# tilmantroester/baryon_painter

Hardware: AMD Instinct MI355X
Metric: cvae_train_tiles_per_sec (higher is better)
Workload: dtype f32; 1 GPU; CVAE fiducial train step (fwd+bwd+Adam), batch 64/GPU of 512x512 tiles, fp32 (BASELINE.json configs[1]); tile=512, batch_per_gpu=64, global_batch=64, parallelism=dp1, batch_norm=single device, optimizer=FlatAdam(lr=1e-3) = torch.optim.Adam arithmetic, fused, schedule=weight gradients on a second HIP stream beside the rest of the backward pass

## Files before the change

baryon_painter_amd/_lib.py:

```python
import ctypes as C
import os

_HERE = os.path.dirname(os.path.abspath(__file__))
LIB_PATH = os.path.join(_HERE, "libbp_hip.so")

BP_OK = 0
BP_EINVAL, BP_EUNSUPPORTED, BP_ELAUNCH, BP_EWORKSPACE = -1, -2, -3, -4
IMPL_AUTO, IMPL_DIRECT, IMPL_MFMA, IMPL_BF16 = 0, 1, 2, 3
IMPL_SHARED = 0x100
IMPL_DEFER = 0x200
PACK_FWD, PACK_BWD = 0, 1
F32, BF16 = 0, 1
F64 = 2
RC_SHIFT_LOG, RC_LOG, RC_SHIFT_LOG_2P, RC_LOG_TANH, RC_X_1PX, RC_INV_X = range(6)


class View(C.Structure):
    _fields_ = [("ptr", C.c_void_p), ("n", C.c_int32), ("h", C.c_int32), ("w", C.c_int32),
                ("c", C.c_int32), ("cstride", C.c_int32), ("coff", C.c_int32), ("dtype", C.c_int32)]


class Pointwise(C.Structure):
    _fields_ = [("scale", C.c_void_p), ("shift", C.c_void_p), ("slope", C.c_void_p)]


class Conv(C.Structure):
    _fields_ = [("transposed", C.c_int32), ("cin", C.c_int32), ("cout", C.c_int32),
                ("k", C.c_int32), ("stride", C.c_int32), ("pad", C.c_int32), ("out_pad", C.c_int32)]


class BnTrain(C.Structure):
    _fields_ = [("count", C.c_double), ("gamma", C.c_void_p), ("beta", C.c_void_p), ("eps", C.c_float),
                ("momentum", C.c_float), ("running_mean", C.c_void_p), ("running_var", C.c_void_p),
                ("num_batches_tracked", C.c_void_p), ("scale", C.c_void_p), ("shift", C.c_void_p),
                ("save_mean", C.c_void_p), ("save_invstd", C.c_void_p)]


class BnBackwardFin(C.Structure):
    _fields_ = [("count", C.c_double), ("gamma", C.c_void_p), ("save_mean", C.c_void_p), ("save_invstd", C.c_void_p),
                ("param_grad_scale", C.c_float), ("dgamma", C.c_void_p), ("dbeta", C.c_void_p), ("coef_abc", C.c_void_p)]


class Latent(C.Structure):
    _fields_ = [("n", C.c_int32), ("L", C.c_int32), ("zc", C.c_int32), ("zh", C.c_int32),
                ("zw", C.c_int32), ("min_z_var", C.c_float)]


class Linear(C.Structure):
    _fields_ = [("in_features", C.c_int32), ("out_features", C.c_int32), ("in_c", C.c_int32), ("in_h", C.c_int32),
                ("in_w", C.c_int32), ("out_c", C.c_int32), ("out_h", C.c_int32), ("out_w", C.c_int32),
                ("has_bias", C.c_int32)]


class Loglik(C.Structure):
    _fields_ = [("n", C.c_int32), ("L", C.c_int32), ("c", C.c_int32), ("h", C.c_int32),
                ("w", C.c_int32), ("mu_softplus", C.c_int32), ("predict_var", C.c_int32),
                ("alpha_var", C.c_float), ("beta_kl", C.c_float), ("likelihood_scaling", C.c_float)]


_P = C.c_void_p
_VP = C.POINTER(View)
_PWP = C.POINTER(Pointwise)
_CP = C.POINTER(Conv)

SIGNATURES = {
    "bp_version": (C.c_int, []),
    "bp_set_option": (C.c_int, [C.c_char_p, C.c_int]),
    "bp_conv_ws_kind": (C.c_int, [_CP, C.c_int, _VP, _VP]),
    "bp_strerror": (C.c_char_p, [C.c_int]),
    "bp_conv_packed_floats": (C.c_int64, [_CP, C.c_int]),
    "bp_conv_kernel_id": (C.c_int, [_CP, C.c_int]),
    "bp_conv_pack": (C.c_int, [_CP, C.c_int, _P, _P, _P]),
    "bp_conv_pack_job_bytes": (C.c_int32, []),
    "bp_conv_pack_job": (C.c_int, [_CP, C.c_int, _P, _P, _P, C.POINTER(C.c_int64)]),
    "bp_conv_pack_jobs": (C.c_int, [_P, _P, C.c_int32, C.c_int64, _P]),
    "bp_conv_bf16_packed_elems": (C.c_int64, [_CP, C.c_int]),
    "bp_conv_bf16_pack": (C.c_int, [_CP, C.c_int, _P, _P, _P]),
    "bp_conv_bf16_supported": (C.c_int, [_CP, C.c_int, _VP, _VP]),
    "bp_conv_forward": (C.c_int, [_CP, _VP, _PWP, _P, _P, _P, _VP, C.c_int, _P]),
    "bp_conv_backward_data": (C.c_int, [_CP, _VP, _P, _P, _VP, C.c_int, _P]),
    "bp_conv_stats_workspace": (C.c_size_t, [_CP, C.c_int, _VP, _VP, C.c_int]),
    "bp_conv_forward_stats": (C.c_int, [_CP, _VP, _PWP, _P, _VP, _P, _P, C.c_size_t, C.c_int, _P]),
    "bp_conv_forward_bn": (C.c_int, [_CP, _VP, _PWP, _P, _VP, _P, C.POINTER(BnTrain), _P, C.c_size_t, C.c_int, _P]),
    "bp_conv_backward_data_stats": (C.c_int, [_CP, _VP, _P, _VP, _VP, _PWP, _P, _P, C.c_size_t, _P]),
    "bp_conv_backward_data_act_workspace": (C.c_size_t, [_CP, _VP, _VP]),
    "bp_conv_backward_data_act": (C.c_int, [_CP, _VP, _P, _VP, _VP, _PWP, _P, _P, C.c_size_t, _P]),
    "bp_conv_backward_weight_workspace": (C.c_size_t, [_CP, _VP, _VP]),
    "bp_conv_backward_weight": (C.c_int, [_CP, _VP, _PWP, _VP, _P, _P, _P, C.c_size_t, C.c_int, _P]),
    "bp_wgrad_defer_begin": (C.c_int, []),
    "bp_wgrad_defer_flush": (C.c_int, [C.c_int, _P]),
    "bp_peer_handle_bytes": (C.c_int, []),
    "bp_peer_max_doubles": (C.c_int, []),
    "bp_peer_create": (C.c_int, [C.c_int, C.c_int, C.POINTER(C.c_void_p), _P]),
    "bp_peer_open": (C.c_int, [_P, _P]),
    "bp_peer_all_reduce": (C.c_int, [_P, _P, C.c_int, C.c_int64, _P]),
    "bp_peer_status": (C.c_int64, [_P]),
    "bp_peer_bind": (C.c_int, [_P]),
    "bp_peer_slots": (C.c_int, []),
    "bp_peer_exchange_check": (C.c_int, [_P, _P, C.c_int, _P]),
    "bp_peer_destroy": (C.c_int, [_P]),
    "bp_channel_sums_workspace": (C.c_size_t, [_VP]),
    "bp_channel_sums": (C.c_int, [_VP, _P, _P, C.c_size_t, _P]),
    "bp_bn_finalize": (C.c_int, [_P, C.c_double, C.c_int32, _P, _P, C.c_float, C.c_float, _P, _P, _P,
                                 _P, _P, _P, _P, _P]),
    "bp_bn_eval_pointwise": (C.c_int, [C.c_int32, _P, _P, _P, _P, C.c_float, _P, _P, _P]),
    "bp_act_backward_workspace": (C.c_size_t, [_VP]),
    "bp_act_backward": (C.c_int, [_VP, _VP, _VP, _PWP, _VP, _VP, _P, _P, C.c_size_t, _P]),
    "bp_act_backward_bn": (C.c_int, [_VP, _VP, _VP, _PWP, _VP, _VP, _P, C.POINTER(BnBackwardFin), _P, C.c_size_t, _P]),
    "bp_bn_backward_finalize": (C.c_int, [_P, C.c_double, C.c_int32, _P, _P, _P, C.c_float, _P, _P, _P, _P]),
    "bp_bn_backward_apply": (C.c_int, [_VP, _VP, _P, _VP, _P]),
    "bp_act_bn_backward_apply": (C.c_int, [_VP, _VP, _VP, _PWP, _VP, _P, _VP, _P]),
    "bp_sums_to_float": (C.c_int, [_P, C.c_int32, _P, _P]),
    "bp_prelu_slope_grad": (C.c_int, [_P, C.c_int32, _P, _P]),
    "bp_residual_forward": (C.c_int, [_VP, _PWP, _VP, _PWP, C.c_float, _VP, _P]),
    "bp_nchw_to_view": (C.c_int, [_P, C.c_int32, _P, C.c_int32, _VP, _P]),
    "bp_view_to_nchw": (C.c_int, [_VP, _PWP, C.c_int32, _P, _P]),
    "bp_fill": (C.c_int, [_P, C.c_int64, C.c_float, _P]),
    "bp_repeat_samples": (C.c_int, [_VP, C.c_int32, _VP, _P]),
    "bp_repeat_samples_adjoint": (C.c_int, [_VP, C.c_int32, _VP, _P]),
    "bp_paint_load": (C.c_int, [_P, C.c_int32, _P, _P, C.c_int32, _VP, _P]),
    "bp_paint_load2": (C.c_int, [_P, C.c_int32, _P, _P, C.c_int32, _VP, _VP, _P]),
    "bp_paint_store": (C.c_int, [_VP, _PWP, C.c_int32, _P, _P, _P]),
    "bp_paint_load_mode": (C.c_int, [C.c_int32, _P, C.c_int32, _P, _P, C.c_int32, _VP, _P]),
    "bp_paint_load2_mode": (C.c_int, [C.c_int32, _P, C.c_int32, _P, _P, C.c_int32, _VP, _VP, _P]),
    "bp_paint_store_mode": (C.c_int, [C.c_int32, _VP, _PWP, C.c_int32, _P, _P, _P]),
    "bp_paint_load_cam": (C.c_int, [_P, C.c_int32, _P, _P, C.c_int32, _VP, _P]),
    "bp_paint_store_cam": (C.c_int, [_VP, _P, _P, _P]),
    "bp_split_scale_workspace": (C.c_size_t, [C.c_int32, C.c_int32, C.c_int32]),
    "bp_split_scale": (C.c_int, [_P, C.c_int32, C.c_int32, C.c_int32, C.c_int32, C.c_int32, _P, _P, _P, C.c_size_t,
                                 _VP, _P]),
    "bp_paint_load_scales2": (C.c_int, [_P, _P, _P, C.c_int32, C.c_int32, C.c_int32, _P, _P, _P, C.c_size_t, _VP, _VP,
                                        _P]),
    "bp_paint_store_scales": (C.c_int, [_VP, _PWP, C.c_int32, C.c_int32, _P, _P, _P]),
    "bp_paint_load_scales2_mode": (C.c_int, [C.c_int32, _P, _P, _P, C.c_int32, C.c_int32, C.c_int32, _P, _P, _P,
                                             C.c_size_t, _VP, _VP, _P]),
    "bp_paint_store_scales_mode": (C.c_int, [C.c_int32, _VP, _PWP, C.c_int32, C.c_int32, _P, _P, _P]),
    "bp_paint_store_fields": (C.c_int, [_P, C.c_int32, C.c_int32, C.c_int32, _VP, _PWP, C.c_int32, _P, _P, _P]),
    "bp_paint_store_moments": (C.c_int, [_P, C.c_int32, C.c_int32, C.c_int32, _VP, _PWP, C.c_int32, _P, C.c_int32, _P, _P,
                                         _P, _P]),
    "bp_philox_normal": (C.c_int, [C.c_uint64, _P, C.c_int32, C.c_int32, C.c_int32, _P, _P]),
    "bp_philox_normal_dev": (C.c_int, [_P, _P, C.c_int32, C.c_int32, C.c_int32, _P, _P]),
    "bp_likelihood_draw": (C.c_int, [_VP, C.c_int32, _VP, _P, _P, _P, _VP, _P]),
    "bp_plane_cut_workspace": (C.c_size_t, [C.c_int32, C.c_int32, C.c_int32]),
    "bp_plane_cut": (C.c_int, [_P, C.c_int32, C.c_int32, C.c_int32, _P, C.c_int32, C.c_int32, C.c_int32, _P,
                               C.c_size_t, _P, _P]),
    "bp_plane_blend": (C.c_int, [_P, C.c_int32, C.c_int32, _P, C.c_int32, C.c_int32, C.c_int32, C.c_int32, _P,
                                 C.c_int32, C.c_double, _P, _P, _P, C.c_int32, C.c_int32, _P]),
    "bp_plane_blend_fields": (C.c_int, [_P, C.c_int32, C.c_int32, C.c_int32, _P, C.c_int32, C.c_int32, C.c_int32,
                                        C.c_int32, _P, C.c_int32, C.c_double, _P, _P, _P, C.c_int32, C.c_int32, _P]),
    "bp_plane_finish": (C.c_int, [_P, _P, C.c_int64, _P, _P]),
    "bp_plane_project_order_workspace": (C.c_size_t, [C.c_int32, C.c_int32, C.c_int32]),
# ... 71 lines not shown
```

baryon_painter_amd/csrc/capi.hip:

```cpp
#include "common.hpp"
#include "kernels.hpp"
#include <cstring>

namespace {

bool conv_ok(const bp_conv* cv) {
  return cv && cv->cin > 0 && cv->cout > 0 && cv->k > 0 && cv->stride > 0 && cv->pad >= 0 && cv->out_pad >= 0 &&
         (cv->transposed == 0 || cv->transposed == 1) && (cv->transposed || cv->out_pad == 0) &&
         cv->out_pad < cv->stride + (cv->stride == 1);
}

bool shapes_ok(const bp_conv* cv, const bp_view* x, const bp_view* y, bool any = false) {
  if (any ? (!bp_view_ok_any(x) || !bp_view_ok_any(y)) : (!bp_view_ok(x) || !bp_view_ok(y))) return false;
  if (x->n != y->n || x->c != cv->cin || y->c != cv->cout) return false;
  return y->h == bp_conv_out_extent(cv, x->h) && y->w == bp_conv_out_extent(cv, x->w) && y->h > 0 && y->w > 0;
}

size_t align256(size_t v) { return (v + 255) & ~(size_t)255; }

}

struct WgradPrivateWs {
  explicit WgradPrivateWs(bool on) { bp_wgrad_private_ws(on); }
  ~WgradPrivateWs() { bp_wgrad_private_ws(false); }
};

extern "C" {

int bp_version(void) { return 100; }

int bp_set_option(const char* name, int value) {
  if (!name) return BP_EINVAL;
  if (!strcmp(name, "bf16_ws")) { bp_bf16_ws_set(value); return BP_OK; }
  if (!strcmp(name, "f32_ws")) { bp_f32_ws_set(value); return BP_OK; }
  if (!strcmp(name, "f32_wgrad_ws")) { bp_f32_wgrad_ws_set(value); return BP_OK; }
  if (!strcmp(name, "bf16_wgrad_ws")) { bp_bf16_wgrad_ws_set(value); return BP_OK; }
  return BP_EUNSUPPORTED;
}

const char* bp_strerror(int code) {
  switch (code) {
    case BP_OK: return "ok";
    case BP_EINVAL: return "invalid argument (null pointer or inconsistent shapes)";
    case BP_EUNSUPPORTED: return "shape not supported by the gfx950 kernels";
    case BP_ELAUNCH: return "kernel launch failed";
    case BP_EWORKSPACE: return "workspace missing or too small";
  }
  return "unknown error";
}

int64_t bp_conv_packed_floats(const bp_conv* cv, int dir) {
  if (!conv_ok(cv) || (dir != BP_PACK_FWD && dir != BP_PACK_BWD)) return -1;
  const ConvGeom g = dir == BP_PACK_FWD ? bp_geom_forward(cv) : bp_geom_backward_data(cv);
  return bp_igemm_packed_floats(g);
}

int bp_conv_kernel_id(const bp_conv* cv, int dir) {
  if (!conv_ok(cv) || (dir != BP_PACK_FWD && dir != BP_PACK_BWD)) return -1;
  return bp_igemm_kernel_id(dir == BP_PACK_FWD ? bp_geom_forward(cv) : bp_geom_backward_data(cv));
}

int bp_conv_pack(const bp_conv* cv, int dir, const float* w_torch, float* packed, void* stream) {
  if (!conv_ok(cv) || !w_torch || !packed || (dir != BP_PACK_FWD && dir != BP_PACK_BWD)) return BP_EINVAL;
  const ConvGeom g = dir == BP_PACK_FWD ? bp_geom_forward(cv) : bp_geom_backward_data(cv);
  return bp_igemm_pack(g, bp_wmap(cv, dir), w_torch, packed, bp_stream(stream));
}

int32_t bp_conv_pack_job_bytes(void) { return (int32_t)bp_igemm_pack_job_bytes(); }

int bp_conv_pack_job(const bp_conv* cv, int dir, const float* w_torch, float* packed, void* job, int64_t* nblocks) {
  if (!conv_ok(cv) || !w_torch || !packed || !job || !nblocks || (dir != BP_PACK_FWD && dir != BP_PACK_BWD))
    return BP_EINVAL;
  const ConvGeom g = dir == BP_PACK_FWD ? bp_geom_forward(cv) : bp_geom_backward_data(cv);
  return bp_igemm_pack_job(g, bp_wmap(cv, dir), w_torch, packed, job, nblocks);
}

int bp_conv_pack_jobs(const void* jobs_dev, const int64_t* first_block_dev, int32_t njobs, int64_t total_blocks,
                      void* stream) {
  if (!jobs_dev || !first_block_dev || njobs < 0 || total_blocks < 0) return BP_EINVAL;
  return bp_igemm_pack_jobs(jobs_dev, first_block_dev, njobs, total_blocks, bp_stream(stream));
}

int64_t bp_conv_bf16_packed_elems(const bp_conv* cv, int dir) {
  if (!conv_ok(cv) || (dir != BP_PACK_FWD && dir != BP_PACK_BWD)) return -1;
  return bp_bf16_packed_elems(dir == BP_PACK_FWD ? bp_geom_forward(cv) : bp_geom_backward_data(cv));
}

int bp_conv_bf16_pack(const bp_conv* cv, int dir, const float* w_torch, void* packed, void* stream) {
  if (!conv_ok(cv) || !w_torch || !packed || (dir != BP_PACK_FWD && dir != BP_PACK_BWD)) return BP_EINVAL;
  const ConvGeom g = dir == BP_PACK_FWD ? bp_geom_forward(cv) : bp_geom_backward_data(cv);
  return bp_bf16_pack(g, bp_wmap(cv, dir), w_torch, packed, bp_stream(stream));
}

int bp_conv_ws_kind(const bp_conv* cv, int dir, const bp_view* in, const bp_view* out) {
  if (!conv_ok(cv) || (dir != BP_PACK_FWD && dir != BP_PACK_BWD) || !bp_view_ok_any(in) || !bp_view_ok_any(out)) return 0;
  const ConvGeom g = dir == BP_PACK_FWD ? bp_geom_forward(cv) : bp_geom_backward_data(cv);
  if (in->dtype == BP_F32 && out->dtype == BP_F32) return bp_f32_ws_ok(g, in, out, nullptr, 0) ? 3 : 0;
  return bp_bf16_ws_ok(g, in, out, nullptr, 0) ? bp_bf16_ws_kind(g) : 0;
}

int bp_conv_bf16_supported(const bp_conv* cv, int dir, const bp_view* in, const bp_view* out) {
  if (!conv_ok(cv) || (dir != BP_PACK_FWD && dir != BP_PACK_BWD)) return 0;
  if ((in && !bp_view_ok_any(in)) || (out && !bp_view_ok_any(out))) return 0;
  return bp_bf16_igemm_ok(dir == BP_PACK_FWD ? bp_geom_forward(cv) : bp_geom_backward_data(cv), in, out) ? 1 : 0;
}

int bp_conv_forward(const bp_conv* cv, const bp_view* x, const bp_pointwise* x_pw, const float* packed_fwd,
                    const float* w_torch, const float* bias, const bp_view* y, int impl, void* stream) {
  if (!conv_ok(cv) || !shapes_ok(cv, x, y, impl == BP_IMPL_BF16)) return BP_EINVAL;
  const ConvGeom g = bp_geom_forward(cv);
  if (impl == BP_IMPL_BF16) {
    if (!packed_fwd) return BP_EINVAL;
    return bp_bf16_igemm_run(g, x, bp_pw(x_pw), packed_fwd, bias, y, bp_stream(stream));
  }
  if (impl == BP_IMPL_AUTO && packed_fwd) {
    const int rc = bp_igemm_run(g, x, bp_pw(x_pw), packed_fwd, bias, y, bp_stream(stream));
    if (rc != BP_EUNSUPPORTED || !w_torch) return rc;
    impl = BP_IMPL_DIRECT;
  }
  if (impl == BP_IMPL_AUTO) impl = BP_IMPL_DIRECT;
  if (impl == BP_IMPL_MFMA) {
    if (!packed_fwd) return BP_EINVAL;
    return bp_igemm_run(g, x, bp_pw(x_pw), packed_fwd, bias, y, bp_stream(stream));
  }
  if (!w_torch) return BP_EINVAL;
  return bp_direct_gather(g, bp_wmap(cv, BP_PACK_FWD), x, bp_pw(x_pw), w_torch, bias, y, bp_stream(stream));
}

size_t bp_conv_stats_workspace(const bp_conv* cv, int dir, const bp_view* x, const bp_view* y, int impl) {
  if (!conv_ok(cv) || !shapes_ok(cv, x, y, impl == BP_IMPL_BF16) || (dir != BP_PACK_FWD && dir != BP_PACK_BWD)) return 0;
  if (impl == BP_IMPL_BF16)
    return dir == BP_PACK_FWD ? bp_bf16_stats_workspace(bp_geom_forward(cv), x, y, 1)
                              : bp_bf16_stats_workspace(bp_geom_backward_data(cv), y, x, 2);
  return dir == BP_PACK_FWD ? bp_igemm_stats_workspace(bp_geom_forward(cv), x, y, 1)
                            : bp_igemm_stats_workspace(bp_geom_backward_data(cv), y, x, 2);
}

int bp_conv_forward_stats(const bp_conv* cv, const bp_view* x, const bp_pointwise* x_pw, const float* packed_fwd,
                          const bp_view* y, double* sums, void* workspace, size_t workspace_bytes, int impl,
                          void* stream) {
  if (!conv_ok(cv) || !shapes_ok(cv, x, y, impl == BP_IMPL_BF16) || !packed_fwd || !sums) return BP_EINVAL;
  const IgemmStatsReq sr{1, nullptr, PW{nullptr, nullptr, nullptr}, sums, workspace, workspace_bytes};
  if (impl == BP_IMPL_BF16)
    return bp_bf16_igemm_run(bp_geom_forward(cv), x, bp_pw(x_pw), packed_fwd, nullptr, y, bp_stream(stream), &sr);
  return bp_igemm_run(bp_geom_forward(cv), x, bp_pw(x_pw), packed_fwd, nullptr, y, bp_stream(stream), &sr);
}

int bp_conv_forward_bn(const bp_conv* cv, const bp_view* x, const bp_pointwise* x_pw, const float* packed_fwd,
                       const bp_view* y, double* sums, const bp_bn_train* bn, void* workspace, size_t workspace_bytes,
                       int impl, void* stream) {
  if (!conv_ok(cv) || !shapes_ok(cv, x, y, impl == BP_IMPL_BF16) || !packed_fwd || !sums || !bn || bn->count <= 0 ||
      !bn->scale || !bn->shift)
    return BP_EINVAL;
  const BnFin fin{bn->count, bn->gamma, bn->beta, bn->eps, bn->momentum, bn->running_mean, bn->running_var,
                  bn->num_batches_tracked, bn->scale, bn->shift, bn->save_mean, bn->save_invstd};
  const IgemmStatsReq sr{1, nullptr, PW{nullptr, nullptr, nullptr}, sums, workspace, workspace_bytes, &fin};
  if (impl == BP_IMPL_BF16)
    return bp_bf16_igemm_run(bp_geom_forward(cv), x, bp_pw(x_pw), packed_fwd, nullptr, y, bp_stream(stream), &sr);
  return bp_igemm_run(bp_geom_forward(cv), x, bp_pw(x_pw), packed_fwd, nullptr, y, bp_stream(stream), &sr);
}

int bp_conv_backward_data_stats(const bp_conv* cv, const bp_view* dy, const float* packed_bwd, const bp_view* dx,
                                const bp_view* x_raw, const bp_pointwise* x_pw, double* sums, void* workspace,
                                size_t workspace_bytes, void* stream) {
  const bool b16 = (dy && dy->dtype == BP_BF16) || (dx && dx->dtype == BP_BF16);
  if (!conv_ok(cv) || !shapes_ok(cv, dx, dy, b16) || !packed_bwd || !sums || !bp_view_ok_any(x_raw)) return BP_EINVAL;
  if (x_raw->n != dx->n || x_raw->h != dx->h || x_raw->w != dx->w || x_raw->c != dx->c) return BP_EINVAL;
  const IgemmStatsReq sr{2, x_raw, bp_pw(x_pw), sums, workspace, workspace_bytes};
  if (b16)
    return bp_bf16_igemm_run(bp_geom_backward_data(cv), dy, PW{nullptr, nullptr, nullptr}, packed_bwd, nullptr, dx,
                             bp_stream(stream), &sr);
  if (!bp_view_ok(x_raw)) return BP_EINVAL;
  return bp_igemm_run(bp_geom_backward_data(cv), dy, PW{nullptr, nullptr, nullptr}, packed_bwd, nullptr, dx,
                      bp_stream(stream), &sr);
}

size_t bp_conv_backward_data_act_workspace(const bp_conv* cv, const bp_view* dy, const bp_view* g) {
  const bool b16 = g && g->dtype == BP_BF16;
  if (!conv_ok(cv) || !shapes_ok(cv, g, dy, b16)) return 0;
  if (b16) return bp_bf16_stats_workspace(bp_geom_backward_data(cv), dy, g, 3);
  return bp_igemm_stats_workspace(bp_geom_backward_data(cv), dy, g, 3);
// ... 101 lines not shown
```

baryon_painter_amd/csrc/conv_flat.hip:

```cpp
#include "common.hpp"
#include "kernels.hpp"
#include <cstdlib>

namespace {

typedef float v4f __attribute__((ext_vector_type(4)));

constexpr int K = 7, CG = 8, CO = 16;
constexpr int NQ = CG / 4;
constexpr int NG = K * NQ;
constexpr int TH = 8, TW = 64;
constexpr int IH = TH + K - 1, IWP = TW + K - 1;
constexpr int PLANE = IH * IWP * 4;
constexpr int NU = IH * IWP * NQ;
constexpr int SL = (NU + 255) / 256;

struct FlatArgs {
  const float* in; int h, w, in_cs, in_co;
  float* out; int out_cs, out_co;
  const float* bias;
  const float* wp;
  PW pw;
  int n, tiles_x, tiles_y, i0, in_vec;
  const float* raw; int raw_cs, raw_co;
  PW spw;
  double* stat;
};

template <bool OUT_VEC, bool STATS2, bool RAW_VEC = true>
__global__ __launch_bounds__(256, 2) void flat_k7_kernel(FlatArgs a) {
  __shared__ __attribute__((aligned(16))) float tile[NQ * PLANE];
  __shared__ double lsum[STATS2 ? 8 * 256 : 1];
  __shared__ double red[STATS2 ? 4 : 1][2][CO];
  const int tid = threadIdx.x, lane = tid & 63;
  const int wave = __builtin_amdgcn_readfirstlane(tid >> 6);
  const int lm = lane & 15, kq = lane >> 4;

  float wreg[K][NG];
#pragma unroll
  for (int u = 0; u < K; ++u)
#pragma unroll
    for (int g = 0; g < NG; ++g) wreg[u][g] = a.wp[((u * NG + g) * 4 + kq) * CO + lm];
  v4f b4 = {0.f, 0.f, 0.f, 0.f};
  if (a.bias) b4 = v4f{a.bias[4 * kq], a.bias[4 * kq + 1], a.bias[4 * kq + 2], a.bias[4 * kq + 3]};

  if constexpr (STATS2) {
#pragma unroll
    for (int q = 0; q < 8; ++q) lsum[q * 256 + tid] = 0.0;
  }
  float ssc[STATS2 ? 4 : 1], ssf[STATS2 ? 4 : 1], ssl[STATS2 ? 4 : 1];
  if constexpr (STATS2) {
#pragma unroll
    for (int q = 0; q < 4; ++q) {
      const bool on = a.spw.scale != nullptr;
      ssc[q] = on ? a.spw.scale[4 * kq + q] : 1.f;
      ssf[q] = on ? a.spw.shift[4 * kq + q] : 0.f;
      ssl[q] = on ? a.spw.slope[4 * kq + q] : 1.f;
    }
  }
  const int q4 = tid % NQ;
  const PW4 p4 = pw4_load(a.pw, q4 * 4, CG);
  const int per_img = a.tiles_x * a.tiles_y;
  const int ntiles = per_img * a.n;
  float4 stage[SL];
  unsigned inside = 0;
  auto fetch = [&](int t) {
    const int n = t / per_img, r = t % per_img;
    const int y0 = (r / a.tiles_x) * TH + a.i0, x0 = (r % a.tiles_x) * TW + a.i0;
    const float* in_n = a.in + (int64_t)n * a.h * a.w * a.in_cs + a.in_co + q4 * 4;
    unsigned in = 0;
#pragma unroll
    for (int i = 0; i < SL; ++i) {
      const int e = tid + i * 256;
      const int pix = e / NQ, col = pix % IWP, row = pix / IWP;
      const int iy = y0 + row, ix = x0 + col;
      if (e < NU && iy >= 0 && iy < a.h && ix >= 0 && ix < a.w) in |= 1u << i;
      const int cy = min(max(iy, 0), a.h - 1), cx = min(max(ix, 0), a.w - 1);
      const float* p = in_n + ((int64_t)cy * a.w + cx) * a.in_cs;
      stage[i] = a.in_vec ? *reinterpret_cast<const float4*>(p) : make_float4(p[0], p[1], p[2], p[3]);
    }
    inside = in;
  };
  auto commit = [&]() {
#pragma unroll
    for (int i = 0; i < SL; ++i) {
// ... 1000 lines not shown
    auto frags = [&](int buf, int g) {
#pragma unroll
      for (int ii = 0; ii < 8; ++ii) {
        const int i = g * 8 + ii, j2 = i % 2, txp = (i / 2) % 8, ty = i / 16;
        const int off = j2 * HPLANE + ((ty * 2 + (txp & 1)) * HHALF + (txp >> 1)) * 4;
        f0[buf][ii] = base[off];
        f1[buf][ii] = base[off + 2 * HHALF * 4];
      }
    };
    frags(0, 0);
#pragma unroll
    for (int g = 0; g < HNW / 8; ++g) {
      if (g + 1 < HNW / 8) frags((g + 1) & 1, g + 1);
      if (g == 8) load_pw();
      __builtin_amdgcn_sched_barrier(0);
#pragma unroll
      for (int i = 0; i < 8; ++i) {
        acc0 = __builtin_amdgcn_mfma_f32_16x16x4f32(wreg[g * 8 + i], f0[g & 1][i], acc0, 0, 0, 0);
        acc1 = __builtin_amdgcn_mfma_f32_16x16x4f32(wreg[g * 8 + i], f1[g & 1][i], acc1, 0, 0, 0);
      }
      if (g < HSL) fetch_unit(g);
      if (g >= 9) finish_unit(g - 9);
      if (g < HSL || g >= 9) {
#pragma unroll
        for (int m = 0; m < 16; ++m) {
          __builtin_amdgcn_sched_group_barrier(0x008, 1, 0);
          __builtin_amdgcn_sched_group_barrier(0x002, 3, 0);
        }
      }
      __builtin_amdgcn_sched_barrier(0);
    }
    float4* xw = reinterpret_cast<float4*>(xch) + ((cur * 4 + rg) * 2) * 64 + lane;
    if (kh == 1) {
      xw[0] = make_float4(acc0[0], acc0[1], acc0[2], acc0[3]);
      xw[64] = make_float4(acc1[0], acc1[1], acc1[2], acc1[3]);
    }
    if (tn < ntiles) commit(tile + (cur ^ 1) * HTILE);
    __syncthreads();
    if (kh == 0) {
      const float4 u0 = xw[0], u1 = xw[64];
      acc0[0] += u0.x; acc0[1] += u0.y; acc0[2] += u0.z; acc0[3] += u0.w;
      acc1[0] += u1.x; acc1[1] += u1.y; acc1[2] += u1.z; acc1[3] += u1.w;
      const int c0 = 4 * (kq & 1);
      if (a.bias) {
#pragma unroll
        for (int q = 0; q < 4; ++q) { const float b = a.bias[c0 + q]; acc0[q] += b; acc1[q] += b; }
      }
      const int ox = ox0 + 2 * lm + (kq >> 1);
      float* out_n = a.out + (int64_t)n * a.h * a.w * a.out_cs + a.out_co + c0;
      if (ox < a.w) {
        if (oy0 < a.h)
          *reinterpret_cast<float4*>(out_n + ((int64_t)oy0 * a.w + ox) * a.out_cs) = make_float4(acc0[0], acc0[1], acc0[2], acc0[3]);
        if (oy0 + 1 < a.h)
          *reinterpret_cast<float4*>(out_n + ((int64_t)(oy0 + 1) * a.w + ox) * a.out_cs) = make_float4(acc1[0], acc1[1], acc1[2], acc1[3]);
      }
    }
    cur ^= 1;
  }
}

struct FlatHPackArgs { const float* w; float* dst; int64_t sa, sb; int flip; };
__global__ void flat_h7_pack_kernel(FlatHPackArgs a) {
  const int i = blockIdx.x * blockDim.x + threadIdx.x;
  if (i >= HKS * 64) return;
  const int m = i % 16, kq = (i / 16) % 4, k = i / 64;
  const int kh = k / HNW, ii = k % HNW;
  const int j = 2 * kh + ii % 2, txp = (ii / 2) % 8, ty = ii / 16;
  const int d = m / 8, co = m % 8, tx = txp - d, c = 4 * j + kq;
  float v = 0.f;
  if (tx >= 0 && tx < HK) {
    const int ky = a.flip ? HK - 1 - ty : ty, kx = a.flip ? HK - 1 - tx : tx;
    v = a.w[c * a.sa + co * a.sb + ky * HK + kx];
  }
  a.dst[i] = v;
}

}

static bool bp_flat_h7_ok(const ConvGeom& g) {
  static const bool off = getenv("BP_NOFLAT") != nullptr || getenv("BP_NOFLATH") != nullptr;
  return !off && g.k == HK && g.stride == 1 && g.pad == HPAD && g.cin_g == HCG && g.cout_g == HCO && g.nphase == 1;
}

static int64_t bp_flat_h7_packed_floats(const ConvGeom&) { return (int64_t)HKS * 64; }

static int bp_flat_h7_pack(const ConvGeom& g, const WeightMap& wm, const float* w_torch, float* packed, hipStream_t st) {
  FlatHPackArgs a{w_torch, packed, wm.sa, wm.sb, g.gather_transposed};
  hipLaunchKernelGGL(flat_h7_pack_kernel, dim3((HKS * 64 + 255) / 256), dim3(256), 0, st, a);
  BP_CHECK_LAUNCH();
  return BP_OK;
}

static int bp_flat_h7_run(const ConvGeom&, const bp_view* in, const PW& pw, const float* packed, const float* bias,
                          const bp_view* out, hipStream_t st, const IgemmStatsReq* sr) {
  if (sr || !bp_view_vec4(out)) return BP_EUNSUPPORTED;
  FlatHArgs a{};
  a.bias = bias;
  a.in = in->ptr; a.h = in->h; a.w = in->w; a.in_cs = in->cstride; a.in_co = in->coff;
  a.out = out->ptr; a.out_cs = out->cstride; a.out_co = out->coff;
  a.wp = packed; a.pw = pw; a.n = in->n; a.in_vec = bp_view_vec4(in) ? 1 : 0;
  a.tiles_x = bp_ceil_div(out->w, HTW); a.tiles_y = bp_ceil_div(out->h, HTH);
  const int64_t ntiles = (int64_t)a.tiles_x * a.tiles_y * a.n;
  if (ntiles > 0x7fffffff) return BP_EUNSUPPORTED;
  hipLaunchKernelGGL(flat_h7_kernel, dim3(flat_g4_grid((int)ntiles)), dim3(GNT), 0, st, a);
  BP_CHECK_LAUNCH();
  return BP_OK;
}

const ConvFamily& bp_family_flat() {
  static const ConvFamily f = {
      "flat", bp_flat_ok, bp_family_id<710000>, bp_flat_packed_floats, bp_flat_pack,
      [](const ConvGeom&, const bp_view*, const bp_view* out, int mode) { return bp_flat_stats_workspace(out, mode); },
      bp_flat_run, false};
  return f;
}
const ConvFamily& bp_family_flat_t4() {
  static const ConvFamily f = {  "flat_t4", bp_flat_t4_ok, bp_family_id<720000>, bp_flat_t4_packed_floats, bp_flat_t4_pack,
                                  bp_family_stats_mode1<bp_flat_t4_stats_workspace>, bp_flat_t4_run, false};
  return f;
}
const ConvFamily& bp_family_flat_g4() {
  static const ConvFamily f = {  "flat_g4", bp_flat_g4_ok, bp_family_id<730000>, bp_flat_g4_packed_floats, bp_flat_g4_pack,
                                  bp_family_stats_mode1<bp_flat_g4_stats_workspace>, bp_flat_g4_run, false};
  return f;
}
const ConvFamily& bp_family_flat_t64() {
  static const ConvFamily f = {  "flat_t64", bp_flat_t64_ok, bp_family_id<740000>, bp_flat_t64_packed_floats,
                                   bp_flat_t64_pack, bp_family_stats_mode1<bp_flat_t64_stats_workspace>, bp_flat_t64_run, false};
  return f;
}
const ConvFamily& bp_family_flat_h7() {
  static const ConvFamily f = {
      "flat_h7", bp_flat_h7_ok, bp_family_id<750000>, bp_flat_h7_packed_floats, bp_flat_h7_pack,
      [](const ConvGeom&, const bp_view*, const bp_view*, int) { return (size_t)0; }, bp_flat_h7_run, false};
  return f;
}
```

baryon_painter_amd/csrc/kernels.hpp:

```cpp
#pragma once
#include "common.hpp"

struct ConvFamily {
  const char* name;
  bool (*ok)(const ConvGeom& g);
  int (*kernel_id)(const ConvGeom& g);
  int64_t (*packed_floats)(const ConvGeom& g);
  int (*pack)(const ConvGeom& g, const WeightMap& wm, const float* w_torch, float* packed, hipStream_t st);
  size_t (*stats_workspace)(const ConvGeom& g, const bp_view* in, const bp_view* out, int mode);
  int (*run)(const ConvGeom& g, const bp_view* in, const PW& pw, const float* packed, const float* bias,
             const bp_view* out, hipStream_t st, const IgemmStatsReq* sr);
  bool batched_pack;
};
template <int ID>
int bp_family_id(const ConvGeom&) { return ID; }
template <size_t (*WS)(const bp_view* out)>
size_t bp_family_stats_mode1(const ConvGeom&, const bp_view*, const bp_view* out, int mode) { return mode == 1 ? WS(out) : 0; }

const ConvFamily& bp_family_enc();
const ConvFamily& bp_family_stem();
const ConvFamily& bp_family_flat();
const ConvFamily& bp_family_flat_t64();
const ConvFamily& bp_family_flat_t4();
const ConvFamily& bp_family_flat_g4();
const ConvFamily& bp_family_flat_h7();
const ConvFamily& bp_family_small();
const ConvFamily& bp_family_tiled();

int64_t bp_igemm_packed_floats(const ConvGeom& g);
int bp_igemm_kernel_id(const ConvGeom& g);
int bp_igemm_pack(const ConvGeom& g, const WeightMap& wm, const float* w_torch, float* packed, hipStream_t st);
int bp_igemm_pack_job(const ConvGeom& g, const WeightMap& wm, const float* w_torch, float* packed, void* job,
                      int64_t* nblocks);
int bp_igemm_run(const ConvGeom& g, const bp_view* in, const PW& pw, const float* packed, const float* bias,
                 const bp_view* out, hipStream_t st, const IgemmStatsReq* stats = nullptr);
size_t bp_igemm_stats_workspace(const ConvGeom& g, const bp_view* in, const bp_view* out, int mode);

size_t bp_igemm_pack_job_bytes();
int bp_igemm_tiled_pack_job(const ConvGeom& g, const WeightMap& wm, const float* w_torch, float* packed, void* job,
                            int64_t* nblocks);
int bp_igemm_pack_jobs(const void* jobs_dev, const int64_t* first_block_dev, int njobs, int64_t total_blocks,
                       hipStream_t st);
size_t bp_stats_rows_bytes(int64_t rows, int C);
int bp_stats_rows_finish(double* ws, int64_t rows, int C, const IgemmStatsReq* sr, hipStream_t st);
int bp_stats_row_stride(int n);
size_t bp_stats_rows_bytes_n(int64_t rows, int n);
int bp_stats_rows_finish_n(double* ws, int64_t rows, int n, const IgemmStatsReq* sr, hipStream_t st);

void bp_f32_ws_set(int v);
bool bp_f32_ws_ok(const ConvGeom& g, const bp_view* in, const bp_view* out, const float* bias, int stats_mode);
size_t bp_f32_ws_stats_workspace(const ConvGeom& g, const bp_view* out);
int bp_f32_ws_run(const ConvGeom& g, const bp_view* in, const PW& pw, const float* packed_tiled, const bp_view* out,
                  hipStream_t st, const IgemmStatsReq* sr);

int bp_direct_gather(const ConvGeom& g, const WeightMap& wm, const bp_view* in, const PW& pw, const float* w_torch,
                     const float* bias, const bp_view* out, hipStream_t st);
int bp_direct_wgrad(const bp_conv* cv, const bp_view* X, const PW& pwx, const bp_view* Y, const PW& pwy, float* dst,
                    hipStream_t st);

size_t bp_wgrad_mfma_workspace(const bp_conv* cv, const bp_view* X, const bp_view* Y);
int bp_wgrad_mfma(const bp_conv* cv, const bp_view* X, const PW& pwx, const bp_view* Y, const PW& pwy, float* dst,
                  void* workspace, size_t workspace_bytes, hipStream_t st, bool shared);
size_t bp_wgrad_bf16_workspace(const bp_conv* cv, const bp_view* X, const bp_view* Y);
int bp_wgrad_bf16_run(const bp_conv* cv, const bp_view* X, const PW& pwx, const bp_view* Y, const PW& pwy, float* dst,
                      void* workspace, size_t workspace_bytes, hipStream_t st);
void bp_wgrad_private_ws(bool on);
int bp_wgrad_defer_begin_impl();
int bp_wgrad_defer_flush_impl(hipStream_t st, int end);

using WgradPartialFn = int(const bp_conv* cv, const bp_view* X, const PW& pwx, const bp_view* Y, const PW& pwy, float* ws,
                           size_t ws_bytes, size_t* need, int* nsplit, int* cxp, int* cyp, hipStream_t st, bool dry);
WgradPartialFn bp_wgrad_ws_f32, bp_wgrad_enc, bp_wgrad_thin, bp_wgrad_small, bp_wgrad_tiles, bp_wgrad_bf16, bp_wgrad_ws_bf16;
void bp_f32_wgrad_ws_set(int v);
void bp_bf16_wgrad_ws_set(int v);
void bp_wgrad_tiles_target(int target);

bool bp_stem_wgrad_ok(const bp_conv* cv, const bp_view* X, const bp_view* Y, const PW& pwy, const float* dbias);
size_t bp_stem_wgrad_workspace(const bp_view* X);
int bp_stem_wgrad(const bp_view* X, const PW& pwx, const bp_view* Y, float* dst, void* workspace, size_t workspace_bytes,
                  hipStream_t st);
bool bp_wgrad_flat_ok(const bp_conv* cv, const bp_view* X, const bp_view* Y, const PW& pwy);
size_t bp_wgrad_flat_workspace(const bp_view* X);
int bp_wgrad_flat(const bp_view* X, const PW& pwx, const bp_view* Y, float* dst, void* workspace, size_t workspace_bytes,
                  hipStream_t st, bool shared);
bool bp_wgrad_flat_s2_ok(const bp_conv* cv, const bp_view* X, const bp_view* Y, const PW& pwx, const PW& pwy);
size_t bp_wgrad_flat_s2_workspace(const bp_view* Y);
int bp_wgrad_flat_s2(const bp_view* X, const PW& pwx, const bp_view* Y, const PW& pwy, float* dst, void* workspace,
                     size_t workspace_bytes, hipStream_t st, bool shared);

bool bp_bf16_igemm_ok(const ConvGeom& g, const bp_view* in, const bp_view* out);
int64_t bp_bf16_packed_elems(const ConvGeom& g);
int bp_bf16_pack(const ConvGeom& g, const WeightMap& wm, const float* w_torch, void* packed, hipStream_t st);
int bp_bf16_igemm_run(const ConvGeom& g, const bp_view* in, const PW& pw, const void* packed, const float* bias,
                      const bp_view* out, hipStream_t st, const IgemmStatsReq* stats = nullptr);
size_t bp_bf16_stats_workspace(const ConvGeom& g, const bp_view* in, const bp_view* out, int mode);

int64_t bp_bf16_flat_packed_elems(const ConvGeom& g);
int bp_bf16_flat_pack(const ConvGeom& g, const WeightMap& wm, const float* w_torch, uint16_t* dst, hipStream_t st);
bool bp_bf16_flat_ok(const ConvGeom& g, const bp_view* in, const bp_view* out, const float* bias, int stats);
size_t bp_bf16_flat_stats_workspace(const ConvGeom& g, const bp_view* in, const bp_view* out, int mode);
int bp_bf16_flat_run(const ConvGeom& g, const bp_view* in, const PW& pw, const uint16_t* packed_flat, const bp_view* out,
                     hipStream_t st, const IgemmStatsReq* sr);

void bp_bf16_ws_set(int v);
int bp_bf16_ws_kind(const ConvGeom& g);
int64_t bp_bf16_ws_packed_elems(const ConvGeom& g);
int bp_bf16_ws_pack(const ConvGeom& g, const WeightMap& wm, const float* w_torch, uint16_t* dst, hipStream_t st);
bool bp_bf16_ws_ok(const ConvGeom& g, const bp_view* in, const bp_view* out, const float* bias, int mode);
// ... 27 lines not shown
```

include/bp_hip.h:

```cpp
#ifndef BP_HIP_H
#define BP_HIP_H

#include <stddef.h>
#include <stdint.h>

#ifdef __cplusplus
extern "C" {
#endif

#define BP_OK 0
#define BP_EINVAL (-1)
#define BP_EUNSUPPORTED (-2)
#define BP_ELAUNCH (-3)
#define BP_EWORKSPACE (-4)

enum { BP_F32 = 0, BP_BF16 = 1 };

typedef struct bp_view {
  float* ptr;
  int32_t n, h, w;
  int32_t c;
  int32_t cstride;
  int32_t coff;
  int32_t dtype;
} bp_view;

typedef struct bp_pointwise {
  const float* scale;
  const float* shift;
  const float* slope;
} bp_pointwise;

typedef struct bp_conv {
  int32_t transposed;
  int32_t cin, cout;
  int32_t k, stride, pad, out_pad;
} bp_conv;

enum { BP_IMPL_AUTO = 0, BP_IMPL_DIRECT = 1, BP_IMPL_MFMA = 2, BP_IMPL_BF16 = 3 };
enum { BP_IMPL_SHARED = 0x100 };
enum { BP_IMPL_DEFER = 0x200 };
enum { BP_PACK_FWD = 0, BP_PACK_BWD = 1 };

int bp_version(void);
int bp_set_option(const char* name, int value);
const char* bp_strerror(int code);


int64_t bp_conv_packed_floats(const bp_conv* cv, int dir);

int bp_conv_kernel_id(const bp_conv* cv, int dir);

int bp_conv_pack(const bp_conv* cv, int dir, const float* w_torch, float* packed, void* stream);

int32_t bp_conv_pack_job_bytes(void);
int bp_conv_pack_job(const bp_conv* cv, int dir, const float* w_torch, float* packed, void* job,
                     int64_t* nblocks);
int bp_conv_pack_jobs(const void* jobs_dev, const int64_t* first_block_dev, int32_t njobs,
                      int64_t total_blocks, void* stream);

int64_t bp_conv_bf16_packed_elems(const bp_conv* cv, int dir);
int bp_conv_ws_kind(const bp_conv* cv, int dir, const bp_view* in, const bp_view* out);
int bp_conv_bf16_pack(const bp_conv* cv, int dir, const float* w_torch, void* packed, void* stream);
int bp_conv_bf16_supported(const bp_conv* cv, int dir, const bp_view* in, const bp_view* out);

int bp_conv_forward(const bp_conv* cv, const bp_view* x, const bp_pointwise* x_pw,
                    const float* packed_fwd, const float* w_torch, const float* bias,
                    const bp_view* y, int impl, void* stream);

int bp_conv_backward_data(const bp_conv* cv, const bp_view* dy, const float* packed_bwd,
                          const float* w_torch, const bp_view* dx, int impl, void* stream);

size_t bp_conv_stats_workspace(const bp_conv* cv, int dir, const bp_view* x, const bp_view* y, int impl);
int bp_conv_forward_stats(const bp_conv* cv, const bp_view* x, const bp_pointwise* x_pw, const float* packed_fwd,
                          const bp_view* y, double* sums, void* workspace, size_t workspace_bytes, int impl,
                          void* stream);
int bp_conv_backward_data_stats(const bp_conv* cv, const bp_view* dy, const float* packed_bwd, const bp_view* dx,
                                const bp_view* x_raw, const bp_pointwise* x_pw, double* sums, void* workspace,
                                size_t workspace_bytes, void* stream);

size_t bp_conv_backward_data_act_workspace(const bp_conv* cv, const bp_view* dy, const bp_view* g);
int bp_conv_backward_data_act(const bp_conv* cv, const bp_view* dy, const float* packed_bwd, const bp_view* g,
                              const bp_view* x_raw, const bp_pointwise* x_pw, double* sums, void* workspace,
                              size_t workspace_bytes, void* stream);

typedef struct bp_bn_train {
  double count;
  const float* gamma; const float* beta;
  float eps, momentum;
  float* running_mean; float* running_var; int64_t* num_batches_tracked;
  float* scale; float* shift;
  double* save_mean; double* save_invstd;
} bp_bn_train;
int bp_conv_forward_bn(const bp_conv* cv, const bp_view* x, const bp_pointwise* x_pw, const float* packed_fwd,
                       const bp_view* y, double* sums, const bp_bn_train* bn, void* workspace, size_t workspace_bytes,
                       int impl, void* stream);

size_t bp_conv_backward_weight_workspace(const bp_conv* cv, const bp_view* x, const bp_view* dy);
int bp_conv_backward_weight(const bp_conv* cv, const bp_view* x, const bp_pointwise* x_pw,
                            const bp_view* dy, float* dw_torch, float* dbias, void* workspace,
                            size_t workspace_bytes, int impl, void* stream);

int bp_wgrad_defer_begin(void);
int bp_wgrad_defer_flush(int end, void* stream);


size_t bp_channel_sums_workspace(const bp_view* x);
int bp_channel_sums(const bp_view* x, double* sums, void* workspace, size_t workspace_bytes,
                    void* stream);

int bp_bn_finalize(const double* sums, double count, int32_t c, const float* gamma,
                   const float* beta, float eps, float momentum, float* running_mean,
                   float* running_var, int64_t* num_batches_tracked, float* scale, float* shift,
                   double* save_mean, double* save_invstd, void* stream);

int bp_bn_eval_pointwise(int32_t c, const float* gamma, const float* beta,
                         const float* running_mean, const float* running_var, float eps,
                         float* scale, float* shift, void* stream);


size_t bp_act_backward_workspace(const bp_view* raw);
int bp_act_backward(const bp_view* dout, const bp_view* dout2, const bp_view* raw,
                    const bp_pointwise* pw, const bp_view* act_out, const bp_view* g,
                    double* sums, void* workspace, size_t workspace_bytes, void* stream);

typedef struct bp_bn_backward_fin {
  double count;
  const float* gamma;
  const double* save_mean; const double* save_invstd;
  float param_grad_scale;
  float* dgamma; float* dbeta;
  double* coef_abc;
} bp_bn_backward_fin;
int bp_act_backward_bn(const bp_view* dout, const bp_view* dout2, const bp_view* raw,
                       const bp_pointwise* pw, const bp_view* act_out, const bp_view* g, double* sums,
                       const bp_bn_backward_fin* fin, void* workspace, size_t workspace_bytes, void* stream);

int bp_bn_backward_finalize(const double* sums, double count, int32_t c, const float* gamma,
                            const double* save_mean, const double* save_invstd,
                            float param_grad_scale, float* dgamma, float* dbeta,
                            double* coef_abc , void* stream);

int bp_bn_backward_apply(const bp_view* g, const bp_view* raw, const double* coef_abc,
                         const bp_view* out, void* stream);

// ... 189 lines not shown
```

Measured before the change: 1615 tiles/s.

## Add row-walking k7 flat conv forward kernel with LDS ring buffer

```diff
diff --git a/baryon_painter_amd/_lib.py b/baryon_painter_amd/_lib.py
--- a/baryon_painter_amd/_lib.py
+++ b/baryon_painter_amd/_lib.py
@@ -67,6 +67,7 @@
     "bp_version": (C.c_int, []),
     "bp_set_option": (C.c_int, [C.c_char_p, C.c_int]),
     "bp_conv_ws_kind": (C.c_int, [_CP, C.c_int, _VP, _VP]),
+    "bp_conv_k7_walk_kind": (C.c_int, [_CP, C.c_int, _VP, _VP]),
     "bp_strerror": (C.c_char_p, [C.c_int]),
     "bp_conv_packed_floats": (C.c_int64, [_CP, C.c_int]),
     "bp_conv_kernel_id": (C.c_int, [_CP, C.c_int]),
diff --git a/baryon_painter_amd/csrc/capi.hip b/baryon_painter_amd/csrc/capi.hip
--- a/baryon_painter_amd/csrc/capi.hip
+++ b/baryon_painter_amd/csrc/capi.hip
@@ -35,6 +35,7 @@
   if (!strcmp(name, "f32_ws")) { bp_f32_ws_set(value); return BP_OK; }
   if (!strcmp(name, "f32_wgrad_ws")) { bp_f32_wgrad_ws_set(value); return BP_OK; }
   if (!strcmp(name, "bf16_wgrad_ws")) { bp_bf16_wgrad_ws_set(value); return BP_OK; }
+  if (!strcmp(name, "f32_k7_walk_fwd")) { bp_f32_k7_walk_fwd_set(value); return BP_OK; }
   return BP_EUNSUPPORTED;
 }
 
@@ -97,6 +98,12 @@
   const ConvGeom g = dir == BP_PACK_FWD ? bp_geom_forward(cv) : bp_geom_backward_data(cv);
   if (in->dtype == BP_F32 && out->dtype == BP_F32) return bp_f32_ws_ok(g, in, out, nullptr, 0) ? 3 : 0;
   return bp_bf16_ws_ok(g, in, out, nullptr, 0) ? bp_bf16_ws_kind(g) : 0;
+}
+
+int bp_conv_k7_walk_kind(const bp_conv* cv, int dir, const bp_view* in, const bp_view* out) {
+  if (!conv_ok(cv) || (dir != BP_PACK_FWD && dir != BP_PACK_BWD) || !bp_view_ok_any(in) || !bp_view_ok_any(out)) return 0;
+  const ConvGeom g = dir == BP_PACK_FWD ? bp_geom_forward(cv) : bp_geom_backward_data(cv);
+  return bp_flat_h7_geom_ok(g) && bp_view_vec4(out) && bp_flat_h7_walk_ok(in, out) ? 1 : 0;
 }
 
 int bp_conv_bf16_supported(const bp_conv* cv, int dir, const bp_view* in, const bp_view* out) {
diff --git a/baryon_painter_amd/csrc/conv_flat.hip b/baryon_painter_amd/csrc/conv_flat.hip
--- a/baryon_painter_amd/csrc/conv_flat.hip
+++ b/baryon_painter_amd/csrc/conv_flat.hip
@@ -1,6 +1,7 @@
 #include "common.hpp"
 #include "kernels.hpp"
 #include <cstdlib>
+#include <type_traits>
 
 namespace {
 
@@ -1167,6 +1168,8 @@
   return !off && g.k == HK && g.stride == 1 && g.pad == HPAD && g.cin_g == HCG && g.cout_g == HCO && g.nphase == 1;
 }
 
+bool bp_flat_h7_geom_ok(const ConvGeom& g) { return bp_flat_h7_ok(g); }
+
 static int64_t bp_flat_h7_packed_floats(const ConvGeom&) { return (int64_t)HKS * 64; }
 
 static int bp_flat_h7_pack(const ConvGeom& g, const WeightMap& wm, const float* w_torch, float* packed, hipStream_t st) {
@@ -1176,9 +1179,215 @@
   return BP_OK;
 }
 
+namespace {
+
+constexpr int RW = 128;
+constexpr int RWP = RW + HK - 1;
+constexpr int RSL = 3;
+constexpr int RSLOTS = RSL * 256;
+
+struct FlatHWArgs {
+  const float* in; int h, w, in_cs, in_co;
+  float* out; int out_cs, out_co;
+  const float* wp;
+  const float* bias;
+  PW pw;
+  int strips, BR, bands;
+};
+
+__global__ __launch_bounds__(256) void flat_h7_walk_kernel(FlatHWArgs a) {
+  __shared__ float4 ring[3 * RSLOTS];
+  const int tid = threadIdx.x, lane = tid & 63;
+  const int wave = __builtin_amdgcn_readfirstlane(tid >> 6);
+  const int lm = lane & 15, kq = lane >> 4;
+  const int item = blockIdx.x;
+  const int strip = item % a.strips, nb = item / a.strips;
+  const int n = nb / a.bands, band = nb % a.bands;
+  const int y0 = band * a.BR, y1 = min(y0 + a.BR, a.h), x0 = strip * RW;
+  const int rs = max(y0 - HPAD, 0), re = min(y1 + HPAD - 1, a.h - 1);
+
+  float wf[HKS];
+  {
+    const float* wsrc = a.wp + ((int64_t)(kq >> 1) * HNW + (kq & 1)) * 64 + lm;
+#pragma unroll
+    for (int s = 0; s < HK * 8; ++s)
+#pragma unroll
+      for (int j = 0; j < 4; ++j) wf[4 * s + j] = wsrc[(2 * s * 4 + j) * 16];
+#pragma unroll
+    for (int s = 0; s < HKS; ++s) asm volatile("" : "+a"(wf[s]));
+  }
+
+  const int q4 = tid & 3;
+  unsigned goff[RSL], keep[RSL];
+#pragma unroll
+  for (int i = 0; i < RSL; ++i) {
+    const int p = (tid + 256 * i) >> 2, x = x0 - HPAD + p;
+    keep[i] = (p < RWP && x >= 0 && x < a.w) ? 0xffffffffu : 0u;
+    goff[i] = (unsigned)(min(max(x, 0), a.w - 1) * a.in_cs + 4 * q4) * 4u;
+  }
+  const char* in_img = reinterpret_cast<const char*>(a.in + (int64_t)n * a.h * a.w * a.in_cs + a.in_co);
+  const unsigned in_row = (unsigned)(a.w * a.in_cs) * 4u;
+  float psc[4], psf[4], psl[4];
+#pragma unroll
+  for (int j = 0; j < 4; ++j) {
+    const bool on = a.pw.scale != nullptr;
+    psc[j] = on ? a.pw.scale[4 * q4 + j] : 1.f;
+    psf[j] = on ? a.pw.shift[4 * q4 + j] : 0.f;
+    psl[j] = on ? a.pw.slope[4 * q4 + j] : 1.f;
+  }
+  float4 raw[RSL];
+  auto load_row = [&](int r) {
+    const char* rowp = in_img + (size_t)((unsigned)r * in_row);
+#pragma unroll
+    for (int i = 0; i < RSL; ++i) raw[i] = *reinterpret_cast<const float4*>(rowp + goff[i]);
+  };
+  auto commit_unit = [&](const float4& rw, int i, int slot) {
+    float v[4] = {rw.x, rw.y, rw.z, rw.w};
+#pragma unroll
+    for (int j = 0; j < 4; ++j) {
+      const float tt = fmaf(v[j], psc[j], psf[j]);
+      v[j] = __uint_as_float(__float_as_uint(tt > 0.f ? tt : tt * psl[j]) & keep[i]);
+    }
+    ring[slot * RSLOTS + tid + 256 * i] = make_float4(v[0], v[1], v[2], v[3]);
+  };
+
+  const int d = kq >> 1, c0 = 4 * (kq & 1);
+  const int ox = x0 + 32 * wave + 2 * lm + d;
+  v4f b4 = {0.f, 0.f, 0.f, 0.f};
+  if (a.bias) b4 = v4f{a.bias[c0], a.bias[c0 + 1], a.bias[c0 + 2], a.bias[c0 + 3]};
+  char* out_img = reinterpret_cast<char*>(a.out + (int64_t)n * a.h * a.w * a.out_cs + a.out_co + c0);
+  const unsigned out_row = (unsigned)(a.w * a.out_cs) * 4u, o_off = (unsigned)(ox * a.out_cs) * 4u;
+  const int fbase = 4 * (32 * wave + 2 * lm) + kq;
+
+  const v4f z4 = {0.f, 0.f, 0.f, 0.f};
+  v4f am[HK], ae0[HK], ae7[HK], e0fin = z4;
+#pragma unroll
+  for (int ty = 0; ty < HK; ++ty) { am[ty] = z4; ae0[ty] = z4; ae7[ty] = z4; }
+  auto e0_step = [&]() {
+    e0fin = ae0[HK - 1];
+#pragma unroll
+    for (int ty = HK - 1; ty > 0; --ty) ae0[ty] = ae0[ty - 1];
+    ae0[0] = z4;
+  };
+  auto epi = [&](auto COND_, int o) {
+    const v4f e = d ? ae7[HK - 1] : e0fin;
+    const v4f v = am[HK - 1] + e + b4;
+    if (!decltype(COND_)::value || (o >= y0 && o < y1 && ox < a.w))
+      *reinterpret_cast<float4*>(out_img + (size_t)((unsigned)o * out_row) + o_off) = make_float4(v[0], v[1], v[2], v[3]);
+#pragma unroll
+    for (int ty = HK - 1; ty > 0; --ty) { am[ty] = am[ty - 1]; ae7[ty] = ae7[ty - 1]; }
+    am[0] = z4; ae7[0] = z4;
+  };
+
+  load_row(rs);
+#pragma unroll
+  for (int i = 0; i < RSL; ++i) commit_unit(raw[i], i, 0);
+  load_row(min(rs + 1, re));
+#pragma unroll
+  for (int i = 0; i < RSL; ++i) commit_unit(raw[i], i, 1);
+  load_row(min(rs + 2, re));
+  __syncthreads();
+
+  float4 xf[2];
+  xf[0] = ring[fbase];
+  int s0 = 0, s1 = 1, s2 = 2;
+  auto row = [&](auto COND_, int r) {
+    float4 rawc[RSL];
+#pragma unroll
+    for (int tx = 0; tx < 8; ++tx) {
+      __builtin_amdgcn_sched_barrier(0);
+      xf[(tx + 1) & 1] = tx < 7 ? ring[s0 * RSLOTS + fbase + 4 * (tx + 1)] : ring[s1 * RSLOTS + fbase];
+      if (tx == 0) epi(COND_, r - HPAD - 1);
+      if (tx == 1) {
+#pragma unroll
+        for (int i = 0; i < RSL; ++i) rawc[i] = raw[i];
+        load_row(min(r + 3, re));
+      }
+      if (tx == 2) e0_step();
+      if (tx >= 3 && tx < 3 + RSL) commit_unit(rawc[tx - 3], tx - 3, s2);
+      const float4 x = xf[tx & 1];
+#pragma unroll
+      for (int j = 0; j < 4; ++j) {
+        const float b = j == 0 ? x.x : j == 1 ? x.y : j == 2 ? x.z : x.w;
+#pragma unroll
+        for (int ty = HK - 1; ty >= 0; --ty) {
+          v4f& acc = tx == 0 ? ae0[ty] : tx == 7 ? ae7[ty] : am[ty];
+          acc = __builtin_amdgcn_mfma_f32_16x16x4f32(wf[(ty * 8 + tx) * 4 + j], b, acc, 0, 0, 0);
+        }
+      }
+      __builtin_amdgcn_sched_group_barrier(0x100, 1, 0);
+#pragma unroll
+      for (int m = 0; m < 4 * HK; ++m) {
+        __builtin_amdgcn_sched_group_barrier(0x008, 1, 0);
+        if (tx == 0) __builtin_amdgcn_sched_group_barrier(0x002, 2, 0);
+        else if (tx < 3 + RSL) __builtin_amdgcn_sched_group_barrier(0x002, 1, 0);
+        if (tx == 0 && m == 20) __builtin_amdgcn_sched_group_barrier(0x040, 1, 0);
+        if (tx == 1 && (m == 4 || m == 8 || m == 12)) __builtin_amdgcn_sched_group_barrier(0x020, 1, 0);
+        if (tx >= 3 && tx < 3 + RSL && m == 26) __builtin_amdgcn_sched_group_barrier(0x200, 1, 0);
+      }
+      __builtin_amdgcn_sched_barrier(0);
+    }
+    asm volatile("s_waitcnt lgkmcnt(0)" ::: "memory");
+    __builtin_amdgcn_s_barrier();
+    asm volatile("" ::: "memory");
+    const int t = s0; s0 = s1; s1 = s2; s2 = t;
+  };
+  int r = rs;
+  const int r_plain = x0 + RW <= a.w ? y0 + HPAD + 1 : re + 1;
+  for (; r <= re && r < r_plain; ++r) row(std::true_type{}, r);
+  for (; r <= re; ++r) row(std::false_type{}, r);
+  epi(std::true_type{}, re - HPAD);
+#pragma unroll
+  for (int k = 1; k <= HPAD; ++k) { e0_step(); epi(std::true_type{}, re - HPAD + k); }
+}
+
+int g_h7_walk_override = -1;
+bool h7_walk_default() {
+  static const bool off = getenv("BP_F32_K7_WALK_FWD") && atoi(getenv("BP_F32_K7_WALK_FWD")) == 0;
+  return !off;
+}
+
+void h7_walk_bands(int n, int h, int strips, int* BR, int* bands) {
+  int br = h;
+  while (br >= 16 && (int64_t)n * strips * bp_ceil_div(h, br) < 256) br = bp_ceil_div(br, 2);
+  *BR = br;
+  *bands = bp_ceil_div(h, br);
+}
+
+}
+
+void bp_f32_k7_walk_fwd_set(int v) { g_h7_walk_override = v; }
+
+bool bp_flat_h7_walk_ok(const bp_view* in, const bp_view* out) {
+  if (!(g_h7_walk_override < 0 ? h7_walk_default() : g_h7_walk_override != 0)) return false;
+  if (!in || !out || in->dtype != BP_F32 || out->dtype != BP_F32 || in->c != HCG || out->c != HCO) return false;
+  if (in->n != out->n || in->h != out->h || in->w != out->w || out->w < RW) return false;
+  if (!bp_view_vec4(in) || !bp_view_vec4(out)) return false;
+  if ((int64_t)in->h * in->w * in->cstride * 4 >= (int64_t)1 << 31 || (int64_t)out->h * out->w * out->cstride * 4 >= (int64_t)1 << 31)
+    return false;
+  int BR, bands;
+  const int strips = bp_ceil_div(out->w, RW);
+  h7_walk_bands(out->n, out->h, strips, &BR, &bands);
+  return (int64_t)out->n * bands * strips <= 0x7fffffff;
+}
+
+static int bp_flat_h7_walk_run(const bp_view* in, const PW& pw, const float* packed, const float* bias, const bp_view* out,
+                               hipStream_t st) {
+  FlatHWArgs a{};
+  a.in = in->ptr; a.h = in->h; a.w = in->w; a.in_cs = in->cstride; a.in_co = in->coff;
+  a.out = out->ptr; a.out_cs = out->cstride; a.out_co = out->coff;
+  a.wp = packed; a.bias = bias; a.pw = pw;
+  a.strips = bp_ceil_div(out->w, RW);
+  h7_walk_bands(out->n, out->h, a.strips, &a.BR, &a.bands);
+  hipLaunchKernelGGL(flat_h7_walk_kernel, dim3((unsigned)(out->n * a.bands * a.strips)), dim3(256), 0, st, a);
+  BP_CHECK_LAUNCH();
+  return BP_OK;
+}
+
 static int bp_flat_h7_run(const ConvGeom&, const bp_view* in, const PW& pw, const float* packed, const float* bias,
                           const bp_view* out, hipStream_t st, const IgemmStatsReq* sr) {
   if (sr || !bp_view_vec4(out)) return BP_EUNSUPPORTED;
+  if (bp_flat_h7_walk_ok(in, out)) return bp_flat_h7_walk_run(in, pw, packed, bias, out, st);
   FlatHArgs a{};
   a.bias = bias;
   a.in = in->ptr; a.h = in->h; a.w = in->w; a.in_cs = in->cstride; a.in_co = in->coff;
diff --git a/baryon_painter_amd/csrc/kernels.hpp b/baryon_painter_amd/csrc/kernels.hpp
--- a/baryon_painter_amd/csrc/kernels.hpp
+++ b/baryon_painter_amd/csrc/kernels.hpp
@@ -24,6 +24,9 @@
 const ConvFamily& bp_family_flat_t4();
 const ConvFamily& bp_family_flat_g4();
 const ConvFamily& bp_family_flat_h7();
+void bp_f32_k7_walk_fwd_set(int v);
+bool bp_flat_h7_geom_ok(const ConvGeom& g);
+bool bp_flat_h7_walk_ok(const bp_view* in, const bp_view* out);
 const ConvFamily& bp_family_small();
 const ConvFamily& bp_family_tiled();
 
diff --git a/include/bp_hip.h b/include/bp_hip.h
--- a/include/bp_hip.h
+++ b/include/bp_hip.h
@@ -61,6 +61,7 @@
 
 int64_t bp_conv_bf16_packed_elems(const bp_conv* cv, int dir);
 int bp_conv_ws_kind(const bp_conv* cv, int dir, const bp_view* in, const bp_view* out);
+int bp_conv_k7_walk_kind(const bp_conv* cv, int dir, const bp_view* in, const bp_view* out);
 int bp_conv_bf16_pack(const bp_conv* cv, int dir, const float* w_torch, void* packed, void* stream);
 int bp_conv_bf16_supported(const bp_conv* cv, int dir, const bp_view* in, const bp_view* out);
 
```

Result: no change. 1628 tiles/s, median of 6 (+0.8%).
